# pipliz/cpuvox

Hardware: NVIDIA B200
Metric: frames/sec @4K, mill 1024^3, BenchmarkPath 60 poses (higher is better)
Workload: dtype f32

## Files before the change

### cpuvox_b200/csrc/raybuffer_kernels.cu

```cuda
#ifdef CVX_EMU
#include "cuda_emu.h"
#else
#include <cuda_runtime.h>
#endif
#include <limits.h>
#include <stdint.h>
#include "device_types.h"

#define FULL_MASK 0xffffffffu
#if defined(CVX_EMU) && defined(CVX_EMU_STATS)
#define EMU_STAT(i) do { if (gl == 0) emu_stats[(int64_t)flat * 16 + (i)]++; } while (0)
#define EMU_STAT_ADD(i, v) do { if (gl == 0) emu_stats[(int64_t)flat * 16 + (i)] += (unsigned long long)(v); } while (0)
extern unsigned long long* emu_stats;
#else
#define EMU_STAT(i) do { } while (0)
#define EMU_STAT_ADD(i, v) do { } while (0)
#endif
#define SKYBOX_ARGB 0x191919FFu

namespace {

struct F3 { float x, y, z; };

__device__ __forceinline__ float lerpf(float a, float b, float t) { return a + t * (b - a); }
// ... 193 lines not shown
}
template <int G>
__device__ __forceinline__ int mark_seen(uint32_t* seen, int a, int b, int gl) {
    int fresh = 0;
    for (int w = (a >> 5) + gl; w <= (b >> 5); w += G) {
        uint32_t m = FULL_MASK;
        if (w == (a >> 5)) m &= mask_from(a);
        if (w == (b >> 5)) m &= mask_to(b);
        const uint32_t old = seen[w], now = old | m;
        fresh += __popc(~old & m);
        seen[w] = now;
    }
    return fresh;
}

struct RowState {
    uint32_t* seen;
    uint32_t* row;
    int orig_min, orig_max;
    int nf_min, nf_max;
    float fb_min, fb_max;
};

__device__ __forceinline__ bool span_would_write(const RowState& rw, int bMin, int bMax) {
    if (!(bMax >= rw.nf_min && bMin <= rw.nf_max)) return false;
    const int a = bMin > rw.nf_min ? bMin : rw.nf_min, b = bMax < rw.nf_max ? bMax : rw.nf_max;
    return a <= b && any_unseen(rw.seen, a, b);
}

__device__ __forceinline__ void reduce_pixel_horizon(RowState& rw, int& bMin, int& bMax) {
    if (bMin <= rw.nf_min) {
        bMin = rw.nf_min;
        if (bMax >= rw.nf_min) {
            rw.nf_min = scan_up(rw.seen, bMax + 1, rw.orig_max);
            rw.fb_min = rw.nf_min - 0.501f;
        }
    }
    if (bMax >= rw.nf_max) {
        bMax = rw.nf_max;
        if (bMin <= rw.nf_max) {
            rw.nf_max = scan_down(rw.seen, bMin - 1, rw.orig_min);
            rw.fb_max = rw.nf_max + 0.501f;
        }
    }
}

struct Acc { unsigned long long dda_steps, columns_nonempty, runs_visited, px_voxel, px_sky; };

#ifndef CVXD_MIN_CTAS_PER_SM
#define CVXD_MIN_CTAS_PER_SM 21
#endif
#if CVXD_MIN_CTAS_PER_SM > 0
#define CVXD_P1_BOUNDS __launch_bounds__(CVXD_THREADS_PER_CTA, CVXD_MIN_CTAS_PER_SM)
#else
#define CVXD_P1_BOUNDS
#endif
template <int G, bool COUNTERS, bool TIMING, bool FAST, bool INV>
__global__ void CVXD_P1_BOUNDS
phase1_kernel(const __grid_constant__ cvxd_world world, const __grid_constant__ cvxd_frame f) {
#ifdef CVX_EMU
    uint32_t* seen_all = emu::g_shared;
#else
    extern __shared__ uint32_t seen_all[];
#endif
    constexpr int GROUPS_PER_CTA = CVXD_THREADS_PER_CTA / G;
    constexpr uint32_t GBITS = G == 32 ? FULL_MASK : ((1u << (G & 31)) - 1u);
    const int lane = threadIdx.x & 31;
    const int gl = lane & (G - 1);
    const int gshift = lane & ~(G - 1);
    const uint32_t gmask = GBITS << gshift;
    const int group = threadIdx.x / G;
    int flat = f.ray_begin + blockIdx.x * GROUPS_PER_CTA + group;
    if (flat >= f.ray_end) return;
    if (f.il_chunk > 0) {
        flat = ((flat / f.il_chunk) * f.il_ranks + f.il_rank) * f.il_chunk + (flat & (f.il_chunk - 1));
        if (flat >= f.total_rays) return;
    }
#define GBALLOT(p) ((__ballot_sync(gmask, (p)) >> gshift) & GBITS)
// ... 2 lines not shown
    long long tAcc[CVXD_TIMING_REGIONS] = {0};
    long long tPrev = TIMING ? clock64() : 0;
    int tCur = 0;
#define STAMP(r) do { if (TIMING) { const long long t_ = clock64(); tAcc[tCur] += t_ - tPrev; tPrev = t_; tCur = (r); } } while (0)

    RaySetup rs;
    setup_ray(world, f, flat, rs);
    if (rs.status < 0) return;
    const cvxd_segment& sg = f.seg[rs.segment];
    const int rowLen = sg.buffer == 0 ? f.height : f.width;
    uint32_t* row = (sg.buffer == 0 ? f.td : f.lr) + (int64_t)(rs.plane_index + sg.ray_index_offset) * rowLen;
    const int seenWords = ((f.width > f.height ? f.width : f.height) + 31) >> 5;

    Acc acc = {0, 0, 0, 0, 0};
    if (COUNTERS && gl == 0) acc.dda_steps = (unsigned long long)rs.lod_steps;
    RowState rw;
    rw.seen = seen_all + group * (seenWords + 9 * G);
    int* scratch = (int*)(rw.seen + seenWords);
    uint32_t* cache = (uint32_t*)(scratch + G);
    rw.row = row;
    rw.orig_min = sg.pix_min; rw.orig_max = sg.pix_max;
    rw.nf_min = rw.orig_min; rw.nf_max = rw.orig_max;
    rw.fb_min = rw.nf_min - 0.501f; rw.fb_max = rw.nf_max + 0.501f;

    if (rs.status == 1) {
        for (int y = rw.orig_min + gl; y <= rw.orig_max; y += G) row[y] = SKYBOX_ARGB;
        if (COUNTERS && gl == 0 && rw.orig_max >= rw.orig_min) acc.px_sky += rw.orig_max - rw.orig_min + 1;
    } else {
        for (int w = gl; w < seenWords; w += G) rw.seen[w] = 0u;
        __syncwarp(gmask);

        Dda ray = rs.dda;
        int lod = rs.lod;
        int voxelScale = 1 << lod;
        const float farClip = f.far_clip;
        float lodMax = f.lod_dist[lod];
        #define worldMaxY (world.dim_y_f)
        const float camY = f.pos_y;
        #define cameraPosYNormalized (f.cam_y_norm)
        constexpr int ITER = INV ? -1 : 1;
        const float EPS = float_epsilon();
        float frustumDirMaxWorld = EPS, frustumDirMinWorld = EPS;

        F3 planeBottom, planeTop, planeDir;
        {
            float top[4], bot[4], dir[4];
            project(f.wts, ray.start_x, worldMaxY, ray.start_z, 1.0f, top);
            project(f.wts, ray.start_x, 0.0f, ray.start_z, 1.0f, bot);
            project(f.wts, ray.dir_x, 0.0f, ray.dir_z, 0.0f, dir);
            const int a = sg.axis_mapped_to_y ? 1 : 0;
            planeBottom = F3{bot[a], bot[2], bot[3]};
            planeTop = F3{top[a], top[2], top[3]};
            planeDir = F3{dir[a], dir[2], dir[3]};
        }
        const int maskX = world.dim_x - 1, maskZ = world.dim_z - 1;

        bool terminated = false;
        bool reachedEnd = false;
        while (!terminated && !reachedEnd) {
            STAMP(1);
            EMU_STAT(0);
            if (ray.dl >= lodMax) {
                dda_next_lod(ray, voxelScale);
                lod++; voxelScale *= 2;
                lodMax = f.lod_dist[lod];
            }
            float myX = ray.tmx, myZ = ray.tmz, xEnd, zEnd;
            {
                float x = ray.tmx, z = ray.tmz;
#pragma unroll
                for (int j = 1; j < G; j++) {
                    x += ray.tdx; z += ray.tdz;
                    if (gl == j) { myX = x; myZ = z; }
                }
                xEnd = x + ray.tdx; zEnd = z + ray.tdz;
            }
            int aK = 0;
            {
                int lo = 0, hi = gl;
#pragma unroll
                for (int it = 0; it < (G == 32 ? 5 : (G == 16 ? 4 : 3)); it++) {
                    const int mid = (lo + hi + 1) >> 1;
                    const float xv = GSHFL(myX, mid > 0 ? mid - 1 : 0), zv = GSHFL(myZ, gl - mid >= 0 ? gl - mid : 0);
                    if (lo < hi) { if (xv < zv) lo = mid; else hi = mid - 1; }
                }
                aK = lo;
            }
            const int bK = gl - aK;
            const float xa = GSHFL(myX, aK), zb = GSHFL(myZ, bK);
            const bool xStep = xa < zb;
            const float myDn = xStep ? xa : zb;
            float myDl = __shfl_up_sync(gmask, myDn, 1, G);
            if (gl == 0) myDl = ray.dl;
            const int cellX = ray.px + aK * ray.sx, cellZ = ray.pz + bK * ray.sz;
            const bool oob = ((cellX & maskX) != cellX) || ((cellZ & maskZ) != cellZ);
            const uint32_t swMask = GBALLOT(gl >= 1 && myDl >= lodMax), oobMask = GBALLOT(oob), farMask = GBALLOT(myDn >= farClip);
            const int kS = swMask ? __ffs(swMask) - 1 : G, kO = oobMask ? __ffs(oobMask) - 1 : G, kF = farMask ? __ffs(farMask) - 1 : G;
            int n, endKind = 0;
            if (kS <= kO && kS <= kF) n = kS;
            else if (kO <= kF) { n = kO; endKind = 1; }
            else { n = kF + 1; endKind = 2; }
            const int myIdx = (cellX >> lod) * world.lods[lod].mul_x + (cellZ >> lod);
            const int myLod = lod;
            if (endKind == 0 && n > 0) {
                const int aN = GSHFL(aK + (xStep ? 1 : 0), n - 1), bN = n - aN;
                const float tx = GSHFL(myX, aN < G ? aN : 0), tz = GSHFL(myZ, bN < G ? bN : 0);
                ray.tmx = aN < G ? tx : xEnd; ray.tmz = bN < G ? tz : zEnd;
                ray.px += aN * ray.sx; ray.pz += bN * ray.sz;
                ray.dl = GSHFL(myDn, n - 1);
                ray.dn = minf_(ray.tmx, ray.tmz);
            }
            uint4 hdr = make_uint4(0, 0, 0, 0);
            if (gl < n) hdr = __ldg(world.lods[myLod].headers + myIdx);
            const bool myNonEmpty = (hdr.y & 0xffffu) != 0u;
            const float myWorldMin = (float)(hdr.y >> 16), myWorldMax = (float)(hdr.z & 0xffffu);
            uint32_t remaining = GBALLOT(myNonEmpty);
            int cellsDone = n + (endKind == 1 ? 1 : 0);

            uint32_t roundCols = 0u;
            uint32_t roundInvalid = 0u;
            int myBase = 0;
            int r_ci = 0, r_sMin = 0, r_sMax = 0, r_cMin = 0, r_cMax = 0, r_capKind = 0;
            bool r_sideClip = false, r_capClip = false;
            float r_eMin = 0.0f, r_eMax = 0.0f;
            int r_len = 0; uint32_t r_capColor = 0u; float bFx = 0.0f, bFy = 0.0f, bFz = 0.0f;
            uint32_t roundHotS = 0u, roundHotC = 0u;
            bool r_solid = false;
            const int myRunCount = (int)(hdr.y & 0xffffu);

            while (remaining) {
                STAMP(2);
                EMU_STAT(1);
                int c;
                float worldBoundsMin = 0.0f, worldBoundsMax = worldMaxY;
                if (frustumDirMaxWorld != EPS) {
                    const float distTop = frustumDirMaxWorld > 0.0f ? myDn : myDl;
                    const float distBot = frustumDirMinWorld < 0.0f ? myDn : myDl;
                    const float newMax = camY + frustumDirMaxWorld * distTop;
                    const float newMin = camY + frustumDirMinWorld * distBot;
                    const bool outOfWorld = newMin > worldMaxY || newMax < 0.0f;
                    const bool culled = myWorldMin > newMax || myWorldMax < newMin;
                    bool inert = false;
// ... 16 lines not shown
                    remaining &= remaining - 1;
                    if (COUNTERS && gl == 0) acc.columns_nonempty++;
                }
                const float distLast = GSHFL(myDl, c);
                const float distNext = GSHFL(myDn, c);
                const int cLod = GSHFL(myLod, c);
                const uint32_t hOff = GSHFL(hdr.x, c);
                const int runCount = GSHFL(myRunCount, c);
                const int cScale = 1 << cLod;

                if (distLast > 2.0f && frustumDirMaxWorld == EPS) {
                    STAMP(3);
                    EMU_STAT(2);
                    const int L = gl & 3;
                    const float dLine = (L & 2) ? distNext : distLast;
                    const F3 pMin = F3{planeBottom.x + planeDir.x * dLine, planeBottom.y + planeDir.y * dLine, planeBottom.z + planeDir.z * dLine};
                    const F3 pMax = F3{planeTop.x + planeDir.x * dLine, planeTop.y + planeDir.y * dLine, planeTop.z + planeDir.z * dLine};
                    const bool A = pMin.x > pMin.z * rw.fb_max, B = pMax.x > pMax.z * rw.fb_max;
                    const bool C = pMin.x < pMin.z * rw.fb_min, D = pMax.x < pMax.z * rw.fb_min;
                    const bool clipped = (A && B) || (!A && !B && C && D);
                    const bool isMax = L & 1;
                    const bool crossHi = isMax ? B : A, crossLo = isMax ? D : C;
                    float myLerp = isMax ? 1.0f : 0.0f;
                    if (crossHi || crossLo) {
                        const float fi = 1.0f / (crossHi ? rw.fb_max : rw.fb_min);
                        const float c0 = cross2(1.0f, fi, pMax.x, pMax.z), c1 = cross2(1.0f, fi, pMin.x, pMin.z);
                        const float num = isMax ? c1 : c0, den = isMax ? c1 - c0 : c0 - c1;
                        const float q = num / den;
                        myLerp = isMax ? q : 1.0f - q;
                    }
                    const F3 pc = lerp3(pMin, pMax, myLerp);
                    const float myProj = pc.x / pc.z;
// ... 16 lines not shown
                        const bool minFromLast = lastMinL < nextMinL, maxFromLast = lastMaxL > nextMaxL;
                        worldBoundsMin = lerpf(0.0f, worldMaxY, minFromLast ? lastMinL : nextMinL); distForMin = minFromLast ? distLast : distNext;
                        worldBoundsMax = lerpf(0.0f, worldMaxY, maxFromLast ? lastMaxL : nextMaxL); distForMax = maxFromLast ? distLast : distNext;
                        if (mxN < mnN) { float t = mxN; mxN = mnN; mnN = t; }
                        if (mxL < mnL) { float t = mxL; mxL = mnL; mnL = t; }
                        clippedMin = minf_(mnL, mnN);
                        clippedMax = maxf_(mxL, mxN);
                    }
                    frustumDirMaxWorld = (worldBoundsMax - camY) / distForMax;
                    frustumDirMinWorld = (worldBoundsMin - camY) / distForMin;
                    worldBoundsMin = floorf(worldBoundsMin);
                    worldBoundsMax = ceilf(worldBoundsMax);
                    const int writableMin = f2i(floorf(clippedMin));
                    const int writableMax = f2i(ceilf(clippedMax));
                    if (writableMax < rw.nf_min || writableMin > rw.nf_max) { terminated = true; cellsDone = c + 1; break; }
                    if (writableMin > rw.nf_min) rw.nf_min = scan_up(rw.seen, writableMin, rw.orig_max);
                    if (writableMax < rw.nf_max) rw.nf_max = scan_down(rw.seen, writableMax, rw.orig_min);
                    if (rw.nf_min > rw.nf_max) { terminated = true; cellsDone = c + 1; break; }
                }

                const uint32_t* colColors = world.lods[cLod].elements + hOff + runCount + 2;

                const bool tall = FAST ? runCount >= G : runCount > G;
                int k0 = 0, yDone = 0;
                bool colStop = false;
                do {
                    STAMP(4);
                    EMU_STAT(3);
                    const int runsHere = tall ? (FAST ? (runCount - k0 < G - 1 ? runCount - k0 : G - 1) : (runCount - k0 < G ? runCount - k0 : G)) : runCount;
                    if (tall || !((roundCols >> c) & 1u)) {
                        EMU_STAT(4);
                        const uint32_t follow = !tall ? remaining : 0u;
// ... 9 lines not shown
                        const uint32_t startMask = __reduce_or_sync(gmask, inRound ? (1u << myBase) : 0u);
                        const int totalRuns = GSHFL(incl, 31 - __clz(roundCols));
                        EMU_STAT_ADD(9, totalRuns);
                        EMU_STAT_ADD(10, __popc(roundCols));
                        EMU_STAT_ADD(11, __popc(consider));
                        __syncwarp(gmask);
                        const int myStart = 31 - __clz(startMask & ((2u << gl) - 1u));
                        const bool hasRun = gl < totalRuns;
                        const int myCol = hasRun ? scratch[myStart] : c;
                        const int k = gl - myStart + (myCol == c ? k0 : 0);
                        __syncwarp(gmask);
                        const float cDl = GSHFL(myDl, myCol), cDn = GSHFL(myDn, myCol);
                        const uint32_t colOff = GSHFL(hdr.x, myCol);
                        const int colRuns = GSHFL(myRunCount, myCol);
                        const uint32_t* colElems = world.lods[cLod].elements + colOff;
                        if (FAST) {
                            const uint32_t colB = GSHFL(hdr.w, myCol);
                            uint2 rec = make_uint2(0u, 0u);
                            if (hasRun) rec = __ldg(world.lods[cLod].bounds + colB + (ITER > 0 ? k : colRuns - k));
                            const int yB = (int)rec.x;
                            const int nextY = __shfl_down_sync(gmask, yB, 1, G);
                            const uint32_t nextEl = __shfl_down_sync(gmask, rec.y, 1, G);
                            const bool laneRun = hasRun && k < colRuns && gl + 1 < totalRuns;
                            const uint32_t el = laneRun ? (ITER > 0 ? rec.y : nextEl) : 0x0000ffffu;
                            r_ci = (int)(short)(el & 0xffffu); r_len = (int)(short)(el >> 16);
                            if (ITER > 0) { r_eMax = (float)yB; r_eMin = (float)nextY; } else { r_eMin = (float)yB; r_eMax = (float)nextY; }

                            STAMP(5);
                            const F3 lMinLast = F3{planeBottom.x + planeDir.x * cDl, planeBottom.y + planeDir.y * cDl, planeBottom.z + planeDir.z * cDl};
                            const F3 lMinNext = F3{planeBottom.x + planeDir.x * cDn, planeBottom.y + planeDir.y * cDn, planeBottom.z + planeDir.z * cDn};
                            const F3 lMaxLast = F3{planeTop.x + planeDir.x * cDl, planeTop.y + planeDir.y * cDl, planeTop.z + planeDir.z * cDl};
                            const F3 lMaxNext = F3{planeTop.x + planeDir.x * cDn, planeTop.y + planeDir.y * cDn, planeTop.z + planeDir.z * cDn};
                            const float portion = world.y_pow2 ? (float)yB * world.inv_dim_y : unlerpf(0.0f, worldMaxY, (float)yB);
                            const F3 Fp = lerp3(lMinLast, lMaxLast, portion), Np = lerp3(lMinNext, lMaxNext, portion);
                            bFx = Fp.x; bFy = Fp.y; bFz = Fp.z;
                            const bool fFront = !(Fp.y <= 0.0f), nFront = !(Np.y <= 0.0f);
                            const int bKind = portion < cameraPosYNormalized ? 1 : (portion > cameraPosYNormalized ? 2 : 0);
                            const float fpx = Fp.x / Fp.z;
                            const int fr = f2i(rintf(fpx));
                            int bcMin = 0, bcMax = 0;
                            if (bKind && fFront && nFront) {
                                const int nr = f2i(rintf(Np.x / Np.z));
                                bcMin = nr; bcMax = fr;
                                if (bcMin > bcMax) { bcMin = fr; bcMax = nr; }
                            }
                            const int flags = (fFront ? 1 : 0) | (nFront ? 2 : 0) | (bKind << 2);
                            const float nextFpx = __shfl_down_sync(gmask, fpx, 1, G);
                            const int nextFlags = __shfl_down_sync(gmask, flags, 1, G);
                            const int nextCMin = __shfl_down_sync(gmask, bcMin, 1, G), nextCMax = __shfl_down_sync(gmask, bcMax, 1, G);
                            const bool nextFront = nextFlags & 1;
                            const int topKind = ITER > 0 ? bKind : (nextFlags >> 2), botKind = ITER > 0 ? (nextFlags >> 2) : bKind;
                            r_capKind = topKind == 1 ? 1 : (botKind == 2 ? 2 : 0);
                            const bool capOwn = (r_capKind == 1) == (ITER > 0);
                            const bool capNFront = capOwn ? nFront : ((nextFlags & 2) != 0);
                            r_sideClip = false; r_capClip = false;
                            const bool solidRun = laneRun && r_ci >= 0;
                            r_solid = solidRun;
                            bool needExact = false;
                            if (solidRun) {
                                if (fFront && nextFront) {
                                    const float fb = ITER > 0 ? nextFpx : fpx, ft = ITER > 0 ? fpx : nextFpx;
                                    const int nextFr = f2i(rintf(nextFpx));
                                    const int rb = ITER > 0 ? nextFr : fr, rt = ITER > 0 ? fr : nextFr;
                                    if (fb > ft) { r_sMin = rt; r_sMax = rb; } else { r_sMin = rb; r_sMax = rt; }
                                    r_sideClip = true;
                                    if (r_capKind) {
                                        if (capNFront) { r_cMin = capOwn ? bcMin : nextCMin; r_cMax = capOwn ? bcMax : nextCMax; r_capClip = true; }
                                        else needExact = true;
                                    }
                                } else if (!fFront && !nextFront) {
                                    if (r_capKind && capNFront) needExact = true;
                                } else needExact = true;
                                if (r_capKind) r_capColor = __ldg(colElems + colRuns + 2 + (r_capKind == 1 ? r_ci : r_ci + r_len - 1));
                            }
                            if (GBALLOT(needExact)) {
                                EMU_STAT(8);
                                const F3 nF = F3{__shfl_down_sync(gmask, Fp.x, 1, G), __shfl_down_sync(gmask, Fp.y, 1, G), __shfl_down_sync(gmask, Fp.z, 1, G)};
                                const F3 nN = F3{__shfl_down_sync(gmask, Np.x, 1, G), __shfl_down_sync(gmask, Np.y, 1, G), __shfl_down_sync(gmask, Np.z, 1, G)};
                                if (needExact) {
                                    F3 frontBottom = ITER > 0 ? nF : Fp, frontTop = ITER > 0 ? Fp : nF;
                                    float uA = (float)r_len, uB = 0.0f;
                                    r_sideClip = false; r_capClip = false;
                                    if (clip_near_u(frontBottom, frontTop, uA, uB)) {
                                        float bfx = frontBottom.x / frontBottom.z, bfy = frontTop.x / frontTop.z;
                                        if (bfx > bfy) { float t = bfx; bfx = bfy; bfy = t; }
                                        r_sMin = f2i(rintf(bfx)); r_sMax = f2i(rintf(bfy));
                                        r_sideClip = true;
                                    }
                                    if (r_capKind) {
                                        F3 secA = capOwn ? Np : nN, secB = r_capKind == 1 ? frontTop : frontBottom;
                                        if (clip_near(secA, secB)) {
                                            r_cMin = f2i(rintf(secA.x / secA.z)); r_cMax = f2i(rintf(secB.x / secB.z));
                                            if (r_cMin > r_cMax) { int t = r_cMin; r_cMin = r_cMax; r_cMax = t; }
                                            r_capClip = true;
                                        }
                                    }
                                }
                            }
                        } else {
                            uint32_t el = 0u;
                            if (hasRun) el = __ldg(colElems + (ITER > 0 ? 1 + k : colRuns - k));
                            r_ci = (int)(short)(el & 0xffffu); r_len = (int)(short)(el >> 16);
                            roundInvalid = GBALLOT(hasRun && r_len == 0);
                            const uint32_t mineUpToMe = ((2u << gl) - 1u) & ~((1u << myStart) - 1u);
                            const bool valid = hasRun && !(roundInvalid & mineUpToMe);
                            r_solid = valid && r_ci >= 0;
                            const int span = valid ? r_len * cScale : 0;
                            int sum = span;
    #pragma unroll
                            for (int o = 1; o < G; o <<= 1) { int t = __shfl_up_sync(gmask, sum, o, G); if (gl >= o) sum += t; }
                            const int before = GSHFL(sum, myStart > 0 ? myStart - 1 : 0);
                            const int inclCol = sum - (myStart > 0 ? before : 0) + (myCol == c ? yDone : 0);
                            if (tall) yDone = GSHFL(inclCol, runsHere - 1);
                            if (ITER > 0) { r_eMax = (float)(world.dim_y - (inclCol - span)); r_eMin = (float)(world.dim_y - inclCol); }
                            else          { r_eMin = (float)(inclCol - span); r_eMax = (float)inclCol; }

                            STAMP(5);
                            const F3 lMinLast = F3{planeBottom.x + planeDir.x * cDl, planeBottom.y + planeDir.y * cDl, planeBottom.z + planeDir.z * cDl};
                            const F3 lMinNext = F3{planeBottom.x + planeDir.x * cDn, planeBottom.y + planeDir.y * cDn, planeBottom.z + planeDir.z * cDn};
                            const F3 lMaxLast = F3{planeTop.x + planeDir.x * cDl, planeTop.y + planeDir.y * cDl, planeTop.z + planeDir.z * cDl};
                            const F3 lMaxNext = F3{planeTop.x + planeDir.x * cDn, planeTop.y + planeDir.y * cDn, planeTop.z + planeDir.z * cDn};
                            r_sideClip = false; r_capClip = false; r_capKind = 0;
                            {
                                float bfx = 0.0f, bfy = 0.0f, uvAx = 0.0f, uvAy = 0.0f, uvBx = 0.0f, uvBy = 0.0f;
                                int capIdx = 0;
                                const float portionBottom = unlerpf(0.0f, worldMaxY, r_eMin);
                                const float portionTop = unlerpf(0.0f, worldMaxY, r_eMax);
                                F3 frontBottom = lerp3(lMinLast, lMaxLast, portionBottom);
                                F3 frontTop = lerp3(lMinLast, lMaxLast, portionTop);
                                if (portionTop < cameraPosYNormalized) { r_capKind = 1; capIdx = r_ci; }
                                else if (portionBottom > cameraPosYNormalized) { r_capKind = 2; capIdx = r_ci + r_len - 1; }
                                uint32_t capColor = 0u;
                                if (r_capKind && valid && r_ci >= 0) capColor = __ldg(colElems + colRuns + 2 + capIdx);
                                float uA = (float)r_len, uB = 0.0f;
                                if (clip_near_u(frontBottom, frontTop, uA, uB)) {
                                    uvAx = 1.0f / frontBottom.z; uvAy = uA / frontBottom.z;
                                    uvBx = 1.0f / frontTop.z;    uvBy = uB / frontTop.z;
                                    bfx = frontBottom.x / frontBottom.z; bfy = frontTop.x / frontTop.z;
                                    if (bfx > bfy) {
                                        float t = bfx; bfx = bfy; bfy = t;
                                        t = uvAx; uvAx = uvBx; uvBx = t;
                                        t = uvAy; uvAy = uvBy; uvBy = t;
                                    }
                                    r_sMin = f2i(rintf(bfx)); r_sMax = f2i(rintf(bfy));
                                    r_sideClip = true;
                                }
                                if (r_capKind) {
                                    const float portion = r_capKind == 1 ? portionTop : portionBottom;
                                    F3 secA = lerp3(lMinNext, lMaxNext, portion), secB = r_capKind == 1 ? frontTop : frontBottom;
                                    if (clip_near(secA, secB)) {
                                        r_cMin = f2i(rintf(secA.x / secA.z)); r_cMax = f2i(rintf(secB.x / secB.z));
                                        if (r_cMin > r_cMax) { int t = r_cMin; r_cMin = r_cMax; r_cMax = t; }
                                        r_capClip = true;
                                    }
                                }
                                cache[0 * G + gl] = __float_as_uint(bfx);  cache[1 * G + gl] = __float_as_uint(bfy);
                                cache[2 * G + gl] = __float_as_uint(uvAx); cache[3 * G + gl] = __float_as_uint(uvAy);
                                cache[4 * G + gl] = __float_as_uint(uvBx); cache[5 * G + gl] = __float_as_uint(uvBy);
                                cache[6 * G + gl] = (uint32_t)r_len;       cache[7 * G + gl] = capColor;
                                __syncwarp(gmask);
                            }
                        }
                        STAMP(6);
                        roundHotS = GBALLOT(r_solid && r_sideClip && span_would_write(rw, r_sMin, r_sMax));
                        roundHotC = GBALLOT(r_solid && r_capClip && span_would_write(rw, r_cMin, r_cMax));
                        STAMP(4);
                    }

                    const int base = GSHFL(myBase, c);
                    const uint32_t colMask = (runsHere >= 32 ? FULL_MASK : ((1u << runsHere) - 1u)) << base;
                    const bool inCol = (colMask >> gl) & 1u;
                    const uint32_t invalidHere = roundInvalid & colMask;
                    const int endValid = invalidHere ? __ffs(invalidHere) - 1 : base + runsHere;
                    const bool solid = inCol && gl < endValid && r_ci >= 0;
                    const bool above = r_eMin > worldBoundsMax, below = r_eMax < worldBoundsMin;
                    const bool isBreak = solid && (ITER > 0 ? (!above && below) : above);
                    const uint32_t breakMask = GBALLOT(isBreak);
                    const int endVisit = breakMask ? __ffs(breakMask) : endValid;
                    if (invalidHere | breakMask) colStop = true;
                    const bool active = solid && gl < endVisit && !above && !below;
                    const bool sideOk = active && r_sideClip;
                    const bool capOk = active && r_capClip &&
                                       (r_capKind == 1 ? !(r_eMax > worldBoundsMax) : !(r_eMin < worldBoundsMin));

                    STAMP(6);
                    uint32_t candS = GBALLOT(sideOk) & roundHotS, candC = GBALLOT(capOk) & roundHotC;
                    int visitedHere = endVisit - base;
                    while (candS | candC) {
                        const int jS = candS ? __ffs(candS) - 1 : 64, jC = candC ? __ffs(candC) - 1 : 64;
                        const bool isCap = jC < jS;
                        const int j = isCap ? jC : jS;
                        if (isCap) candC &= candC - 1u; else candS &= candS - 1u;
                        int bMin = GSHFL(isCap ? r_cMin : r_sMin, j), bMax = GSHFL(isCap ? r_cMax : r_sMax, j);
                        EMU_STAT(5);
                        STAMP(8);
                        if (!span_would_write(rw, bMin, bMax)) { STAMP(6); continue; }
                        EMU_STAT(6);
                        if (isCap) EMU_STAT(7);
                        STAMP(9);
                        reduce_pixel_horizon(rw, bMin, bMax);
                        STAMP(10);
                        if (isCap) {
                            const uint32_t color = FAST ? GSHFL(r_capColor, j) : cache[7 * G + j];
                            for (int y = bMin + gl; y <= bMax; y += G)
                                if (!((rw.seen[y >> 5] >> (y & 31)) & 1u)) row[y] = color;
                        } else {
                            STAMP(11);
                            float jbfx, jbfy, jAx, jAy, jBx, jBy;
                            int jLen;
                            const int jCi = GSHFL(r_ci, j);
                            if (FAST) {
                                jLen = GSHFL(r_len, j);
                                jbfx = jbfy = jAx = jAy = jBx = jBy = 0.0f;
                                if (jLen > 1) {
                                    const F3 pj = F3{GSHFL(bFx, j), GSHFL(bFy, j), GSHFL(bFz, j)}, pn = F3{GSHFL(bFx, j + 1), GSHFL(bFy, j + 1), GSHFL(bFz, j + 1)};
                                    F3 frontBottom = ITER > 0 ? pn : pj, frontTop = ITER > 0 ? pj : pn;
                                    float uA = (float)jLen, uB = 0.0f;
                                    clip_near_u(frontBottom, frontTop, uA, uB);
                                    jAx = 1.0f / frontBottom.z; jAy = uA / frontBottom.z;
                                    jBx = 1.0f / frontTop.z;    jBy = uB / frontTop.z;
                                    jbfx = frontBottom.x / frontBottom.z; jbfy = frontTop.x / frontTop.z;
                                    if (jbfx > jbfy) {
                                        float t = jbfx; jbfx = jbfy; jbfy = t;
                                        t = jAx; jAx = jBx; jBx = t;
                                        t = jAy; jAy = jBy; jBy = t;
                                    }
                                }
                            } else {
                                jbfx = __uint_as_float(cache[0 * G + j]); jbfy = __uint_as_float(cache[1 * G + j]);
                                jAx = __uint_as_float(cache[2 * G + j]); jAy = __uint_as_float(cache[3 * G + j]);
                                jBx = __uint_as_float(cache[4 * G + j]); jBy = __uint_as_float(cache[5 * G + j]);
                                jLen = (int)cache[6 * G + j];
                            }
                            STAMP(12);
                            for (int y = bMin + gl; y <= bMax; y += G) {
                                if (!((rw.seen[y >> 5] >> (y & 31)) & 1u)) {
                                    int idx = jCi;
                                    if (!FAST || jLen > 1) {
                                        float l = unlerpf(jbfx, jbfy, (float)y);
                                        float wx = lerpf(jAx, jBx, l), wy = lerpf(jAy, jBy, l);
                                        float u = wy / wx;
                                        idx = max(0, min(jLen - 1, f2i(floorf(u)))) + jCi;
                                    }
                                    row[y] = __ldg(colColors + idx);
                                }
                            }
                        }
// ... 4 lines not shown
                        STAMP(6);
                        frustumDirMaxWorld = EPS;
                        if (rw.nf_min > rw.nf_max) { terminated = true; visitedHere = j + 1 - base; break; }
                    }
                    if (COUNTERS && gl == 0) acc.runs_visited += visitedHere;
                    if (tall) { k0 += FAST ? G - 1 : G; roundCols = 0u; }
                } while (tall && k0 < runCount && !colStop && !terminated);
                STAMP(4);
                if (terminated) { cellsDone = c + 1; break; }
            }
            if (COUNTERS && gl == 0) acc.dda_steps += cellsDone;
            if (endKind != 0) reachedEnd = true;
        }
        STAMP(7);
        __syncwarp(gmask);
        for (int y = rw.orig_min + gl; y <= rw.orig_max; y += G)
            if (!((rw.seen[y >> 5] >> (y & 31)) & 1u)) row[y] = SKYBOX_ARGB;
        if (COUNTERS) {
            for (int w = (rw.orig_min >> 5) + gl; w <= (rw.orig_max >> 5); w += G) {
                uint32_t m = FULL_MASK;
                if (w == (rw.orig_min >> 5)) m &= mask_from(rw.orig_min);
                if (w == (rw.orig_max >> 5)) m &= mask_to(rw.orig_max);
                acc.px_sky += __popc(~rw.seen[w] & m);
            }
        }
    }

    STAMP(0);
    if (TIMING && f.timing && gl == 0)
        for (int i = 0; i < CVXD_TIMING_REGIONS; i++) f.timing[(int64_t)flat * CVXD_TIMING_REGIONS + i] = tAcc[i];
#undef STAMP
    if (COUNTERS && f.counters) {
        if (acc.dda_steps) atomicAdd(&f.counters->dda_steps, acc.dda_steps);
        if (acc.columns_nonempty) atomicAdd(&f.counters->columns_nonempty, acc.columns_nonempty);
        if (acc.runs_visited) atomicAdd(&f.counters->runs_visited, acc.runs_visited);
        if (acc.px_voxel) atomicAdd(&f.counters->px_voxel, acc.px_voxel);
        if (acc.px_sky) atomicAdd(&f.counters->px_sky, acc.px_sky);
        if (gl == 0) atomicAdd(&f.counters->rays, 1ull);
    }
#undef GBALLOT
#undef GSHFL
#undef worldMaxY
#undef cameraPosYNormalized
}

struct P2Pixel { uint32_t color; bool owned; };

struct P2Seg {
    float e1x, e1y, e2x, e2y, det;
    float scale, offset, rowsF;
    int off01, rc, flatBase;
};
__device__ __forceinline__ P2Seg p2_seg(const cvxd_blit& p, int k) {
    P2Seg g;
    g.e1x = p.seg[k].max_screen[0] - p.vp_x; g.e1y = p.seg[k].max_screen[1] - p.vp_y;
    g.e2x = p.seg[k].min_screen[0] - p.vp_x; g.e2y = p.seg[k].min_screen[1] - p.vp_y;
    g.det = g.e1x * g.e2y - g.e1y * g.e2x;
// ... 275 lines not shown
}

__global__ void fill_kernel(uint32_t* dst, uint32_t value, int64_t n) {
    int64_t i = (int64_t)blockIdx.x * blockDim.x + threadIdx.x;
    int64_t stride = (int64_t)gridDim.x * blockDim.x;
    for (; i < n; i += stride) dst[i] = value;
}

}

#ifndef CVX_EMU
template <int G>
static cudaError_t launch_phase1_g(const cvxd_world& world, const cvxd_frame& frame, int n, cudaStream_t stream) {
    constexpr int groupsPerCta = CVXD_THREADS_PER_CTA / G;
    const int blocks = (n + groupsPerCta - 1) / groupsPerCta;
    const int seenWords = ((frame.width > frame.height ? frame.width : frame.height) + 31) >> 5;
    const size_t smem = (size_t)groupsPerCta * (seenWords + 9 * G) * sizeof(uint32_t);
    const bool fast = world.regular && !frame.general_path;
#define CVXD_P1(C, T, F) do { \
        if (frame.inverse) phase1_kernel<G, C, T, F, true><<<blocks, CVXD_THREADS_PER_CTA, smem, stream>>>(world, frame); \
        else               phase1_kernel<G, C, T, F, false><<<blocks, CVXD_THREADS_PER_CTA, smem, stream>>>(world, frame); } while (0)
    if (frame.timing) {
        if constexpr (G != 32) return cudaErrorInvalidValue;
        else { if (fast) CVXD_P1(false, true, true); else CVXD_P1(false, true, false); }
    }
    else if (frame.counters) { if (fast) CVXD_P1(true, false, true); else CVXD_P1(true, false, false); }
    else { if (fast) CVXD_P1(false, false, true); else CVXD_P1(false, false, false); }
#undef CVXD_P1
    return cudaGetLastError();
}

cudaError_t cvxd_launch_phase1(const cvxd_world& world, const cvxd_frame& frame, int group_size, cudaStream_t stream) {
// ... 50 lines not shown
```

Before: 1410.

## Spill per-group ray state to shared memory and pack spans to cut registers

Moves the per-group DDA ray state, projected plane vectors, row pointer and original bounds into a shared-memory P1Group struct, and packs span min/max and element fields into 16-bit pairs. Per-run base points and cap colours move into the shared cache instead of living in registers. Together with raising the minimum CTAs per SM in the launch bounds from 21 to 32, this is meant to lower register pressure and raise occupancy. The cost is extra shared-memory traffic on every loop iteration, additional warp syncs when the ray state is written back, and possible register spills under the tighter bound.

Result: faster. 1505 (median of 6 runs) (+6.7%).

```diff
diff --git a/cpuvox_b200/csrc/raybuffer_kernels.cu b/cpuvox_b200/csrc/raybuffer_kernels.cu
--- a/cpuvox_b200/csrc/raybuffer_kernels.cu
+++ b/cpuvox_b200/csrc/raybuffer_kernels.cu
@@ -231,13 +231,33 @@
     return fresh;
 }
 
+struct P1Group {
+    Dda ray;
+    F3 planeBottom, planeTop, planeDir;
+    uint32_t* row;
+    int orig_min, orig_max;
+};
+
+static size_t phase1_smem_bytes(int G, int width, int height) {
+    const int seenWords = ((width > height ? width : height) + 31) >> 5;
+    return (size_t)(CVXD_THREADS_PER_CTA / G) * (sizeof(P1Group) + (size_t)(seenWords + 8 * G) * sizeof(uint32_t));
+}
+
 struct RowState {
     uint32_t* seen;
-    uint32_t* row;
-    int orig_min, orig_max;
+    const P1Group* grp;
     int nf_min, nf_max;
     float fb_min, fb_max;
 };
+
+__device__ __forceinline__ int el_ci(uint32_t e) { return (int)(short)(e & 0xffffu); }
+__device__ __forceinline__ int el_len(uint32_t e) { return (int)(short)(e >> 16); }
+__device__ __forceinline__ uint32_t span_pack(int lo, int hi) {
+    lo = max(-32768, min(32767, lo)); hi = max(-32768, min(32767, hi));
+    return ((uint32_t)lo & 0xffffu) | ((uint32_t)hi << 16);
+}
+__device__ __forceinline__ int span_lo(uint32_t s) { return (int)(short)(s & 0xffffu); }
+__device__ __forceinline__ int span_hi(uint32_t s) { return (int)s >> 16; }
 
 __device__ __forceinline__ bool span_would_write(const RowState& rw, int bMin, int bMax) {
     if (!(bMax >= rw.nf_min && bMin <= rw.nf_max)) return false;
@@ -249,14 +269,14 @@
     if (bMin <= rw.nf_min) {
         bMin = rw.nf_min;
         if (bMax >= rw.nf_min) {
-            rw.nf_min = scan_up(rw.seen, bMax + 1, rw.orig_max);
+            rw.nf_min = scan_up(rw.seen, bMax + 1, rw.grp->orig_max);
             rw.fb_min = rw.nf_min - 0.501f;
         }
     }
     if (bMax >= rw.nf_max) {
         bMax = rw.nf_max;
         if (bMin <= rw.nf_max) {
-            rw.nf_max = scan_down(rw.seen, bMin - 1, rw.orig_min);
+            rw.nf_max = scan_down(rw.seen, bMin - 1, rw.grp->orig_min);
             rw.fb_max = rw.nf_max + 0.501f;
         }
     }
@@ -265,7 +285,7 @@
 struct Acc { unsigned long long dda_steps, columns_nonempty, runs_visited, px_voxel, px_sky; };
 
 #ifndef CVXD_MIN_CTAS_PER_SM
-#define CVXD_MIN_CTAS_PER_SM 21
+#define CVXD_MIN_CTAS_PER_SM 32
 #endif
 #if CVXD_MIN_CTAS_PER_SM > 0
 #define CVXD_P1_BOUNDS __launch_bounds__(CVXD_THREADS_PER_CTA, CVXD_MIN_CTAS_PER_SM)
@@ -276,9 +296,9 @@
 __global__ void CVXD_P1_BOUNDS
 phase1_kernel(const __grid_constant__ cvxd_world world, const __grid_constant__ cvxd_frame f) {
 #ifdef CVX_EMU
-    uint32_t* seen_all = emu::g_shared;
+    uint32_t* smem_all = emu::g_shared;
 #else
-    extern __shared__ uint32_t seen_all[];
+    extern __shared__ __align__(16) uint32_t smem_all[];
 #endif
     constexpr int GROUPS_PER_CTA = CVXD_THREADS_PER_CTA / G;
     constexpr uint32_t GBITS = G == 32 ? FULL_MASK : ((1u << (G & 31)) - 1u);
@@ -311,57 +331,57 @@
 
     Acc acc = {0, 0, 0, 0, 0};
     if (COUNTERS && gl == 0) acc.dda_steps = (unsigned long long)rs.lod_steps;
+    P1Group& gs = reinterpret_cast<P1Group*>(smem_all)[group];
     RowState rw;
-    rw.seen = seen_all + group * (seenWords + 9 * G);
+    rw.seen = reinterpret_cast<uint32_t*>(reinterpret_cast<P1Group*>(smem_all) + GROUPS_PER_CTA) + group * (seenWords + 8 * G);
+    rw.grp = &gs;
     int* scratch = (int*)(rw.seen + seenWords);
     uint32_t* cache = (uint32_t*)(scratch + G);
-    rw.row = row;
-    rw.orig_min = sg.pix_min; rw.orig_max = sg.pix_max;
-    rw.nf_min = rw.orig_min; rw.nf_max = rw.orig_max;
+    const int origMin = sg.pix_min, origMax = sg.pix_max;
+    rw.nf_min = origMin; rw.nf_max = origMax;
     rw.fb_min = rw.nf_min - 0.501f; rw.fb_max = rw.nf_max + 0.501f;
 
     if (rs.status == 1) {
-        for (int y = rw.orig_min + gl; y <= rw.orig_max; y += G) row[y] = SKYBOX_ARGB;
-        if (COUNTERS && gl == 0 && rw.orig_max >= rw.orig_min) acc.px_sky += rw.orig_max - rw.orig_min + 1;
+        for (int y = origMin + gl; y <= origMax; y += G) row[y] = SKYBOX_ARGB;
+        if (COUNTERS && gl == 0 && origMax >= origMin) acc.px_sky += origMax - origMin + 1;
     } else {
         for (int w = gl; w < seenWords; w += G) rw.seen[w] = 0u;
-        __syncwarp(gmask);
-
-        Dda ray = rs.dda;
+        gs.ray = rs.dda;
+        gs.row = row;
+        gs.orig_min = origMin; gs.orig_max = origMax;
+
         int lod = rs.lod;
-        int voxelScale = 1 << lod;
-        const float farClip = f.far_clip;
-        float lodMax = f.lod_dist[lod];
         #define worldMaxY (world.dim_y_f)
-        const float camY = f.pos_y;
+        #define farClip (f.far_clip)
+        #define camY (f.pos_y)
         #define cameraPosYNormalized (f.cam_y_norm)
         constexpr int ITER = INV ? -1 : 1;
         const float EPS = float_epsilon();
         float frustumDirMaxWorld = EPS, frustumDirMinWorld = EPS;
 
-        F3 planeBottom, planeTop, planeDir;
         {
             float top[4], bot[4], dir[4];
-            project(f.wts, ray.start_x, worldMaxY, ray.start_z, 1.0f, top);
-            project(f.wts, ray.start_x, 0.0f, ray.start_z, 1.0f, bot);
-            project(f.wts, ray.dir_x, 0.0f, ray.dir_z, 0.0f, dir);
-            const int a = sg.axis_mapped_to_y ? 1 : 0;
-            planeBottom = F3{bot[a], bot[2], bot[3]};
-            planeTop = F3{top[a], top[2], top[3]};
-            planeDir = F3{dir[a], dir[2], dir[3]};
-        }
-        const int maskX = world.dim_x - 1, maskZ = world.dim_z - 1;
+            project(f.wts, rs.dda.start_x, worldMaxY, rs.dda.start_z, 1.0f, top);
+            project(f.wts, rs.dda.start_x, 0.0f, rs.dda.start_z, 1.0f, bot);
+            project(f.wts, rs.dda.dir_x, 0.0f, rs.dda.dir_z, 0.0f, dir);
+            const bool a = sg.axis_mapped_to_y;
+            gs.planeBottom = F3{a ? bot[1] : bot[0], bot[2], bot[3]};
+            gs.planeTop = F3{a ? top[1] : top[0], top[2], top[3]};
+            gs.planeDir = F3{a ? dir[1] : dir[0], dir[2], dir[3]};
+        }
+        __syncwarp(gmask);
 
         bool terminated = false;
         bool reachedEnd = false;
         while (!terminated && !reachedEnd) {
             STAMP(1);
             EMU_STAT(0);
-            if (ray.dl >= lodMax) {
-                dda_next_lod(ray, voxelScale);
-                lod++; voxelScale *= 2;
-                lodMax = f.lod_dist[lod];
+            Dda ray = gs.ray;
+            if (ray.dl >= f.lod_dist[lod]) {
+                dda_next_lod(ray, 1 << lod);
+                lod++;
             }
+            const float lodMax = f.lod_dist[lod];
             float myX = ray.tmx, myZ = ray.tmz, xEnd, zEnd;
             {
                 float x = ray.tmx, z = ray.tmz;
@@ -390,7 +410,7 @@
             float myDl = __shfl_up_sync(gmask, myDn, 1, G);
             if (gl == 0) myDl = ray.dl;
             const int cellX = ray.px + aK * ray.sx, cellZ = ray.pz + bK * ray.sz;
-            const bool oob = ((cellX & maskX) != cellX) || ((cellZ & maskZ) != cellZ);
+            const bool oob = ((cellX & (world.dim_x - 1)) != cellX) || ((cellZ & (world.dim_z - 1)) != cellZ);
             const uint32_t swMask = GBALLOT(gl >= 1 && myDl >= lodMax), oobMask = GBALLOT(oob), farMask = GBALLOT(myDn >= farClip);
             const int kS = swMask ? __ffs(swMask) - 1 : G, kO = oobMask ? __ffs(oobMask) - 1 : G, kF = farMask ? __ffs(farMask) - 1 : G;
             int n, endKind = 0;
@@ -406,6 +426,8 @@
                 ray.px += aN * ray.sx; ray.pz += bN * ray.sz;
                 ray.dl = GSHFL(myDn, n - 1);
                 ray.dn = minf_(ray.tmx, ray.tmz);
+                __syncwarp(gmask);
+                gs.ray = ray;
             }
             uint4 hdr = make_uint4(0, 0, 0, 0);
             if (gl < n) hdr = __ldg(world.lods[myLod].headers + myIdx);
@@ -417,12 +439,10 @@
             uint32_t roundCols = 0u;
             uint32_t roundInvalid = 0u;
             int myBase = 0;
-            int r_ci = 0, r_sMin = 0, r_sMax = 0, r_cMin = 0, r_cMax = 0, r_capKind = 0;
-            bool r_sideClip = false, r_capClip = false;
+            uint32_t r_el = 0u, r_side = 0u, r_cap = 0u;
+            int r_capKind = 0;
             float r_eMin = 0.0f, r_eMax = 0.0f;
-            int r_len = 0; uint32_t r_capColor = 0u; float bFx = 0.0f, bFy = 0.0f, bFz = 0.0f;
             uint32_t roundHotS = 0u, roundHotC = 0u;
-            bool r_solid = false;
             const int myRunCount = (int)(hdr.y & 0xffffu);
 
             while (remaining) {
@@ -469,8 +489,9 @@
                     EMU_STAT(2);
                     const int L = gl & 3;
                     const float dLine = (L & 2) ? distNext : distLast;
-                    const F3 pMin = F3{planeBottom.x + planeDir.x * dLine, planeBottom.y + planeDir.y * dLine, planeBottom.z + planeDir.z * dLine};
-                    const F3 pMax = F3{planeTop.x + planeDir.x * dLine, planeTop.y + planeDir.y * dLine, planeTop.z + planeDir.z * dLine};
+                    const F3 pB = gs.planeBottom, pT = gs.planeTop, pD = gs.planeDir;
+                    const F3 pMin = F3{pB.x + pD.x * dLine, pB.y + pD.y * dLine, pB.z + pD.z * dLine};
+                    const F3 pMax = F3{pT.x + pD.x * dLine, pT.y + pD.y * dLine, pT.z + pD.z * dLine};
                     const bool A = pMin.x > pMin.z * rw.fb_max, B = pMax.x > pMax.z * rw.fb_max;
                     const bool C = pMin.x < pMin.z * rw.fb_min, D = pMax.x < pMax.z * rw.fb_min;
                     const bool clipped = (A && B) || (!A && !B && C && D);
@@ -517,8 +538,8 @@
                     const int writableMin = f2i(floorf(clippedMin));
                     const int writableMax = f2i(ceilf(clippedMax));
                     if (writableMax < rw.nf_min || writableMin > rw.nf_max) { terminated = true; cellsDone = c + 1; break; }
-                    if (writableMin > rw.nf_min) rw.nf_min = scan_up(rw.seen, writableMin, rw.orig_max);
-                    if (writableMax < rw.nf_max) rw.nf_max = scan_down(rw.seen, writableMax, rw.orig_min);
+                    if (writableMin > rw.nf_min) rw.nf_min = scan_up(rw.seen, writableMin, gs.orig_max);
+                    if (writableMax < rw.nf_max) rw.nf_max = scan_down(rw.seen, writableMax, gs.orig_min);
                     if (rw.nf_min > rw.nf_max) { terminated = true; cellsDone = c + 1; break; }
                 }
 
@@ -558,6 +579,7 @@
                         const uint32_t colOff = GSHFL(hdr.x, myCol);
                         const int colRuns = GSHFL(myRunCount, myCol);
                         const uint32_t* colElems = world.lods[cLod].elements + colOff;
+                        bool solidRun = false, sideClip = false, capClip = false;
                         if (FAST) {
                             const uint32_t colB = GSHFL(hdr.w, myCol);
                             uint2 rec = make_uint2(0u, 0u);
@@ -567,89 +589,92 @@
                             const uint32_t nextEl = __shfl_down_sync(gmask, rec.y, 1, G);
                             const bool laneRun = hasRun && k < colRuns && gl + 1 < totalRuns;
                             const uint32_t el = laneRun ? (ITER > 0 ? rec.y : nextEl) : 0x0000ffffu;
-                            r_ci = (int)(short)(el & 0xffffu); r_len = (int)(short)(el >> 16);
+                            r_el = el;
+                            const int ci = el_ci(el), len = el_len(el);
                             if (ITER > 0) { r_eMax = (float)yB; r_eMin = (float)nextY; } else { r_eMin = (float)yB; r_eMax = (float)nextY; }
 
                             STAMP(5);
-                            const F3 lMinLast = F3{planeBottom.x + planeDir.x * cDl, planeBottom.y + planeDir.y * cDl, planeBottom.z + planeDir.z * cDl};
-                            const F3 lMinNext = F3{planeBottom.x + planeDir.x * cDn, planeBottom.y + planeDir.y * cDn, planeBottom.z + planeDir.z * cDn};
-                            const F3 lMaxLast = F3{planeTop.x + planeDir.x * cDl, planeTop.y + planeDir.y * cDl, planeTop.z + planeDir.z * cDl};
-                            const F3 lMaxNext = F3{planeTop.x + planeDir.x * cDn, planeTop.y + planeDir.y * cDn, planeTop.z + planeDir.z * cDn};
+                            const F3 pB = gs.planeBottom, pT = gs.planeTop, pD = gs.planeDir;
+                            const F3 lMinLast = F3{pB.x + pD.x * cDl, pB.y + pD.y * cDl, pB.z + pD.z * cDl};
+                            const F3 lMinNext = F3{pB.x + pD.x * cDn, pB.y + pD.y * cDn, pB.z + pD.z * cDn};
+                            const F3 lMaxLast = F3{pT.x + pD.x * cDl, pT.y + pD.y * cDl, pT.z + pD.z * cDl};
+                            const F3 lMaxNext = F3{pT.x + pD.x * cDn, pT.y + pD.y * cDn, pT.z + pD.z * cDn};
                             const float portion = world.y_pow2 ? (float)yB * world.inv_dim_y : unlerpf(0.0f, worldMaxY, (float)yB);
                             const F3 Fp = lerp3(lMinLast, lMaxLast, portion), Np = lerp3(lMinNext, lMaxNext, portion);
-                            bFx = Fp.x; bFy = Fp.y; bFz = Fp.z;
+                            cache[0 * G + gl] = __float_as_uint(Fp.x); cache[1 * G + gl] = __float_as_uint(Fp.y); cache[2 * G + gl] = __float_as_uint(Fp.z);
                             const bool fFront = !(Fp.y <= 0.0f), nFront = !(Np.y <= 0.0f);
                             const int bKind = portion < cameraPosYNormalized ? 1 : (portion > cameraPosYNormalized ? 2 : 0);
                             const float fpx = Fp.x / Fp.z;
                             const int fr = f2i(rintf(fpx));
-                            int bcMin = 0, bcMax = 0;
+                            uint32_t bcSpan = 0u;
                             if (bKind && fFront && nFront) {
                                 const int nr = f2i(rintf(Np.x / Np.z));
-                                bcMin = nr; bcMax = fr;
-                                if (bcMin > bcMax) { bcMin = fr; bcMax = nr; }
+                                bcSpan = nr > fr ? span_pack(fr, nr) : span_pack(nr, fr);
                             }
                             const int flags = (fFront ? 1 : 0) | (nFront ? 2 : 0) | (bKind << 2);
                             const float nextFpx = __shfl_down_sync(gmask, fpx, 1, G);
                             const int nextFlags = __shfl_down_sync(gmask, flags, 1, G);
-                            const int nextCMin = __shfl_down_sync(gmask, bcMin, 1, G), nextCMax = __shfl_down_sync(gmask, bcMax, 1, G);
+                            const uint32_t nextCSpan = __shfl_down_sync(gmask, bcSpan, 1, G);
                             const bool nextFront = nextFlags & 1;
                             const int topKind = ITER > 0 ? bKind : (nextFlags >> 2), botKind = ITER > 0 ? (nextFlags >> 2) : bKind;
                             r_capKind = topKind == 1 ? 1 : (botKind == 2 ? 2 : 0);
                             const bool capOwn = (r_capKind == 1) == (ITER > 0);
                             const bool capNFront = capOwn ? nFront : ((nextFlags & 2) != 0);
-                            r_sideClip = false; r_capClip = false;
-                            const bool solidRun = laneRun && r_ci >= 0;
-                            r_solid = solidRun;
+                            solidRun = laneRun && ci >= 0;
                             bool needExact = false;
+                            uint32_t capColor = 0u;
                             if (solidRun) {
                                 if (fFront && nextFront) {
                                     const float fb = ITER > 0 ? nextFpx : fpx, ft = ITER > 0 ? fpx : nextFpx;
                                     const int nextFr = f2i(rintf(nextFpx));
                                     const int rb = ITER > 0 ? nextFr : fr, rt = ITER > 0 ? fr : nextFr;
-                                    if (fb > ft) { r_sMin = rt; r_sMax = rb; } else { r_sMin = rb; r_sMax = rt; }
-                                    r_sideClip = true;
+                                    r_side = fb > ft ? span_pack(rt, rb) : span_pack(rb, rt);
+                                    sideClip = true;
                                     if (r_capKind) {
-                                        if (capNFront) { r_cMin = capOwn ? bcMin : nextCMin; r_cMax = capOwn ? bcMax : nextCMax; r_capClip = true; }
+                                        if (capNFront) { r_cap = capOwn ? bcSpan : nextCSpan; capClip = true; }
                                         else needExact = true;
                                     }
                                 } else if (!fFront && !nextFront) {
                                     if (r_capKind && capNFront) needExact = true;
                                 } else needExact = true;
-                                if (r_capKind) r_capColor = __ldg(colElems + colRuns + 2 + (r_capKind == 1 ? r_ci : r_ci + r_len - 1));
+                                if (r_capKind) capColor = __ldg(colElems + colRuns + 2 + (r_capKind == 1 ? ci : ci + len - 1));
                             }
+                            cache[6 * G + gl] = capColor;
                             if (GBALLOT(needExact)) {
                                 EMU_STAT(8);
                                 const F3 nF = F3{__shfl_down_sync(gmask, Fp.x, 1, G), __shfl_down_sync(gmask, Fp.y, 1, G), __shfl_down_sync(gmask, Fp.z, 1, G)};
                                 const F3 nN = F3{__shfl_down_sync(gmask, Np.x, 1, G), __shfl_down_sync(gmask, Np.y, 1, G), __shfl_down_sync(gmask, Np.z, 1, G)};
                                 if (needExact) {
                                     F3 frontBottom = ITER > 0 ? nF : Fp, frontTop = ITER > 0 ? Fp : nF;
-                                    float uA = (float)r_len, uB = 0.0f;
-                                    r_sideClip = false; r_capClip = false;
+                                    float uA = (float)len, uB = 0.0f;
+                                    sideClip = false; capClip = false;
                                     if (clip_near_u(frontBottom, frontTop, uA, uB)) {
                                         float bfx = frontBottom.x / frontBottom.z, bfy = frontTop.x / frontTop.z;
                                         if (bfx > bfy) { float t = bfx; bfx = bfy; bfy = t; }
-                                        r_sMin = f2i(rintf(bfx)); r_sMax = f2i(rintf(bfy));
-                                        r_sideClip = true;
+                                        r_side = span_pack(f2i(rintf(bfx)), f2i(rintf(bfy)));
+                                        sideClip = true;
                                     }
                                     if (r_capKind) {
                                         F3 secA = capOwn ? Np : nN, secB = r_capKind == 1 ? frontTop : frontBottom;
                                         if (clip_near(secA, secB)) {
-                                            r_cMin = f2i(rintf(secA.x / secA.z)); r_cMax = f2i(rintf(secB.x / secB.z));
-                                            if (r_cMin > r_cMax) { int t = r_cMin; r_cMin = r_cMax; r_cMax = t; }
-                                            r_capClip = true;
+                                            const int a = f2i(rintf(secA.x / secA.z)), b = f2i(rintf(secB.x / secB.z));
+                                            r_cap = a > b ? span_pack(b, a) : span_pack(a, b);
+                                            capClip = true;
                                         }
                                     }
                                 }
                             }
+                            __syncwarp(gmask);
                         } else {
                             uint32_t el = 0u;
                             if (hasRun) el = __ldg(colElems + (ITER > 0 ? 1 + k : colRuns - k));
-                            r_ci = (int)(short)(el & 0xffffu); r_len = (int)(short)(el >> 16);
-                            roundInvalid = GBALLOT(hasRun && r_len == 0);
+                            r_el = el;
+                            const int ci = el_ci(el), len = el_len(el);
+                            roundInvalid = GBALLOT(hasRun && len == 0);
                             const uint32_t mineUpToMe = ((2u << gl) - 1u) & ~((1u << myStart) - 1u);
                             const bool valid = hasRun && !(roundInvalid & mineUpToMe);
-                            r_solid = valid && r_ci >= 0;
-                            const int span = valid ? r_len * cScale : 0;
+                            solidRun = valid && ci >= 0;
+                            const int span = valid ? len * cScale : 0;
                             int sum = span;
     #pragma unroll
                             for (int o = 1; o < G; o <<= 1) { int t = __shfl_up_sync(gmask, sum, o, G); if (gl >= o) sum += t; }
@@ -660,11 +685,12 @@
                             else          { r_eMin = (float)(inclCol - span); r_eMax = (float)inclCol; }
 
                             STAMP(5);
-                            const F3 lMinLast = F3{planeBottom.x + planeDir.x * cDl, planeBottom.y + planeDir.y * cDl, planeBottom.z + planeDir.z * cDl};
-                            const F3 lMinNext = F3{planeBottom.x + planeDir.x * cDn, planeBottom.y + planeDir.y * cDn, planeBottom.z + planeDir.z * cDn};
-                            const F3 lMaxLast = F3{planeTop.x + planeDir.x * cDl, planeTop.y + planeDir.y * cDl, planeTop.z + planeDir.z * cDl};
-                            const F3 lMaxNext = F3{planeTop.x + planeDir.x * cDn, planeTop.y + planeDir.y * cDn, planeTop.z + planeDir.z * cDn};
-                            r_sideClip = false; r_capClip = false; r_capKind = 0;
+                            const F3 pB = gs.planeBottom, pT = gs.planeTop, pD = gs.planeDir;
+                            const F3 lMinLast = F3{pB.x + pD.x * cDl, pB.y + pD.y * cDl, pB.z + pD.z * cDl};
+                            const F3 lMinNext = F3{pB.x + pD.x * cDn, pB.y + pD.y * cDn, pB.z + pD.z * cDn};
+                            const F3 lMaxLast = F3{pT.x + pD.x * cDl, pT.y + pD.y * cDl, pT.z + pD.z * cDl};
+                            const F3 lMaxNext = F3{pT.x + pD.x * cDn, pT.y + pD.y * cDn, pT.z + pD.z * cDn};
+                            r_capKind = 0;
                             {
                                 float bfx = 0.0f, bfy = 0.0f, uvAx = 0.0f, uvAy = 0.0f, uvBx = 0.0f, uvBy = 0.0f;
                                 int capIdx = 0;
@@ -672,11 +698,11 @@
                                 const float portionTop = unlerpf(0.0f, worldMaxY, r_eMax);
                                 F3 frontBottom = lerp3(lMinLast, lMaxLast, portionBottom);
                                 F3 frontTop = lerp3(lMinLast, lMaxLast, portionTop);
-                                if (portionTop < cameraPosYNormalized) { r_capKind = 1; capIdx = r_ci; }
-                                else if (portionBottom > cameraPosYNormalized) { r_capKind = 2; capIdx = r_ci + r_len - 1; }
+                                if (portionTop < cameraPosYNormalized) { r_capKind = 1; capIdx = ci; }
+                                else if (portionBottom > cameraPosYNormalized) { r_capKind = 2; capIdx = ci + len - 1; }
                                 uint32_t capColor = 0u;
-                                if (r_capKind && valid && r_ci >= 0) capColor = __ldg(colElems + colRuns + 2 + capIdx);
-                                float uA = (float)r_len, uB = 0.0f;
+                                if (r_capKind && solidRun) capColor = __ldg(colElems + colRuns + 2 + capIdx);
+                                float uA = (float)len, uB = 0.0f;
                                 if (clip_near_u(frontBottom, frontTop, uA, uB)) {
                                     uvAx = 1.0f / frontBottom.z; uvAy = uA / frontBottom.z;
                                     uvBx = 1.0f / frontTop.z;    uvBy = uB / frontTop.z;
@@ -686,28 +712,28 @@
                                         t = uvAx; uvAx = uvBx; uvBx = t;
                                         t = uvAy; uvAy = uvBy; uvBy = t;
                                     }
-                                    r_sMin = f2i(rintf(bfx)); r_sMax = f2i(rintf(bfy));
-                                    r_sideClip = true;
+                                    r_side = span_pack(f2i(rintf(bfx)), f2i(rintf(bfy)));
+                                    sideClip = true;
                                 }
                                 if (r_capKind) {
                                     const float portion = r_capKind == 1 ? portionTop : portionBottom;
                                     F3 secA = lerp3(lMinNext, lMaxNext, portion), secB = r_capKind == 1 ? frontTop : frontBottom;
                                     if (clip_near(secA, secB)) {
-                                        r_cMin = f2i(rintf(secA.x / secA.z)); r_cMax = f2i(rintf(secB.x / secB.z));
-                                        if (r_cMin > r_cMax) { int t = r_cMin; r_cMin = r_cMax; r_cMax = t; }
-                                        r_capClip = true;
+                                        const int a = f2i(rintf(secA.x / secA.z)), b = f2i(rintf(secB.x / secB.z));
+                                        r_cap = a > b ? span_pack(b, a) : span_pack(a, b);
+                                        capClip = true;
                                     }
                                 }
                                 cache[0 * G + gl] = __float_as_uint(bfx);  cache[1 * G + gl] = __float_as_uint(bfy);
                                 cache[2 * G + gl] = __float_as_uint(uvAx); cache[3 * G + gl] = __float_as_uint(uvAy);
                                 cache[4 * G + gl] = __float_as_uint(uvBx); cache[5 * G + gl] = __float_as_uint(uvBy);
-                                cache[6 * G + gl] = (uint32_t)r_len;       cache[7 * G + gl] = capColor;
+                                cache[6 * G + gl] = capColor;
                                 __syncwarp(gmask);
                             }
                         }
                         STAMP(6);
-                        roundHotS = GBALLOT(r_solid && r_sideClip && span_would_write(rw, r_sMin, r_sMax));
-                        roundHotC = GBALLOT(r_solid && r_capClip && span_would_write(rw, r_cMin, r_cMax));
+                        roundHotS = GBALLOT(solidRun && sideClip && span_would_write(rw, span_lo(r_side), span_hi(r_side)));
+                        roundHotC = GBALLOT(solidRun && capClip && span_would_write(rw, span_lo(r_cap), span_hi(r_cap)));
                         STAMP(4);
                     }
 
@@ -716,26 +742,25 @@
                     const bool inCol = (colMask >> gl) & 1u;
                     const uint32_t invalidHere = roundInvalid & colMask;
                     const int endValid = invalidHere ? __ffs(invalidHere) - 1 : base + runsHere;
-                    const bool solid = inCol && gl < endValid && r_ci >= 0;
+                    const bool solid = inCol && gl < endValid && el_ci(r_el) >= 0;
                     const bool above = r_eMin > worldBoundsMax, below = r_eMax < worldBoundsMin;
                     const bool isBreak = solid && (ITER > 0 ? (!above && below) : above);
                     const uint32_t breakMask = GBALLOT(isBreak);
                     const int endVisit = breakMask ? __ffs(breakMask) : endValid;
                     if (invalidHere | breakMask) colStop = true;
                     const bool active = solid && gl < endVisit && !above && !below;
-                    const bool sideOk = active && r_sideClip;
-                    const bool capOk = active && r_capClip &&
-                                       (r_capKind == 1 ? !(r_eMax > worldBoundsMax) : !(r_eMin < worldBoundsMin));
+                    const bool capOk = active && (r_capKind == 1 ? !(r_eMax > worldBoundsMax) : !(r_eMin < worldBoundsMin));
 
                     STAMP(6);
-                    uint32_t candS = GBALLOT(sideOk) & roundHotS, candC = GBALLOT(capOk) & roundHotC;
+                    uint32_t candS = GBALLOT(active) & roundHotS, candC = GBALLOT(capOk) & roundHotC;
                     int visitedHere = endVisit - base;
                     while (candS | candC) {
                         const int jS = candS ? __ffs(candS) - 1 : 64, jC = candC ? __ffs(candC) - 1 : 64;
                         const bool isCap = jC < jS;
                         const int j = isCap ? jC : jS;
                         if (isCap) candC &= candC - 1u; else candS &= candS - 1u;
-                        int bMin = GSHFL(isCap ? r_cMin : r_sMin, j), bMax = GSHFL(isCap ? r_cMax : r_sMax, j);
+                        const uint32_t span = GSHFL(isCap ? r_cap : r_side, j);
+                        int bMin = span_lo(span), bMax = span_hi(span);
                         EMU_STAT(5);
                         STAMP(8);
                         if (!span_would_write(rw, bMin, bMax)) { STAMP(6); continue; }
@@ -744,20 +769,21 @@
                         STAMP(9);
                         reduce_pixel_horizon(rw, bMin, bMax);
                         STAMP(10);
+                        uint32_t* const row = gs.row;
                         if (isCap) {
-                            const uint32_t color = FAST ? GSHFL(r_capColor, j) : cache[7 * G + j];
+                            const uint32_t color = cache[6 * G + j];
                             for (int y = bMin + gl; y <= bMax; y += G)
                                 if (!((rw.seen[y >> 5] >> (y & 31)) & 1u)) row[y] = color;
                         } else {
                             STAMP(11);
                             float jbfx, jbfy, jAx, jAy, jBx, jBy;
-                            int jLen;
-                            const int jCi = GSHFL(r_ci, j);
+                            const uint32_t jEl = GSHFL(r_el, j);
+                            const int jCi = el_ci(jEl), jLen = el_len(jEl);
                             if (FAST) {
-                                jLen = GSHFL(r_len, j);
                                 jbfx = jbfy = jAx = jAy = jBx = jBy = 0.0f;
                                 if (jLen > 1) {
-                                    const F3 pj = F3{GSHFL(bFx, j), GSHFL(bFy, j), GSHFL(bFz, j)}, pn = F3{GSHFL(bFx, j + 1), GSHFL(bFy, j + 1), GSHFL(bFz, j + 1)};
+                                    const F3 pj = F3{__uint_as_float(cache[0 * G + j]), __uint_as_float(cache[1 * G + j]), __uint_as_float(cache[2 * G + j])};
+                                    const F3 pn = F3{__uint_as_float(cache[0 * G + j + 1]), __uint_as_float(cache[1 * G + j + 1]), __uint_as_float(cache[2 * G + j + 1])};
                                     F3 frontBottom = ITER > 0 ? pn : pj, frontTop = ITER > 0 ? pj : pn;
                                     float uA = (float)jLen, uB = 0.0f;
                                     clip_near_u(frontBottom, frontTop, uA, uB);
@@ -774,7 +800,6 @@
                                 jbfx = __uint_as_float(cache[0 * G + j]); jbfy = __uint_as_float(cache[1 * G + j]);
                                 jAx = __uint_as_float(cache[2 * G + j]); jAy = __uint_as_float(cache[3 * G + j]);
                                 jBx = __uint_as_float(cache[4 * G + j]); jBy = __uint_as_float(cache[5 * G + j]);
-                                jLen = (int)cache[6 * G + j];
                             }
                             STAMP(12);
                             for (int y = bMin + gl; y <= bMax; y += G) {
@@ -809,13 +834,15 @@
         }
         STAMP(7);
         __syncwarp(gmask);
-        for (int y = rw.orig_min + gl; y <= rw.orig_max; y += G)
+        uint32_t* const row = gs.row;
+        const int origMin = gs.orig_min, origMax = gs.orig_max;
+        for (int y = origMin + gl; y <= origMax; y += G)
             if (!((rw.seen[y >> 5] >> (y & 31)) & 1u)) row[y] = SKYBOX_ARGB;
         if (COUNTERS) {
-            for (int w = (rw.orig_min >> 5) + gl; w <= (rw.orig_max >> 5); w += G) {
+            for (int w = (origMin >> 5) + gl; w <= (origMax >> 5); w += G) {
                 uint32_t m = FULL_MASK;
-                if (w == (rw.orig_min >> 5)) m &= mask_from(rw.orig_min);
-                if (w == (rw.orig_max >> 5)) m &= mask_to(rw.orig_max);
+                if (w == (origMin >> 5)) m &= mask_from(origMin);
+                if (w == (origMax >> 5)) m &= mask_to(origMax);
                 acc.px_sky += __popc(~rw.seen[w] & m);
             }
         }
@@ -836,6 +863,8 @@
 #undef GBALLOT
 #undef GSHFL
 #undef worldMaxY
+#undef farClip
+#undef camY
 #undef cameraPosYNormalized
 }
 
@@ -1141,8 +1170,7 @@
 static cudaError_t launch_phase1_g(const cvxd_world& world, const cvxd_frame& frame, int n, cudaStream_t stream) {
     constexpr int groupsPerCta = CVXD_THREADS_PER_CTA / G;
     const int blocks = (n + groupsPerCta - 1) / groupsPerCta;
-    const int seenWords = ((frame.width > frame.height ? frame.width : frame.height) + 31) >> 5;
-    const size_t smem = (size_t)groupsPerCta * (seenWords + 9 * G) * sizeof(uint32_t);
+    const size_t smem = phase1_smem_bytes(G, frame.width, frame.height);
     const bool fast = world.regular && !frame.general_path;
 #define CVXD_P1(C, T, F) do { \
         if (frame.inverse) phase1_kernel<G, C, T, F, true><<<blocks, CVXD_THREADS_PER_CTA, smem, stream>>>(world, frame); \
```
